# thu-nics/Rad-NeRF

Hardware: AMD Instinct MI355X
Metric: million samples/s fwd+bwd, 8192 rays, model_zoo_size=2; rgb L∞ vs ref (higher is better)
Workload: dtype f16/f32

## Files before the change

rad-nerf_amd/csrc/field.hip:

```cpp
#include "rn_field.h"
#include "rn_bin.h"
#pragma clang fp contract(off)

static int g_field_dbg = 0;
static uint64_t g_level_pairing = 0;
__device__ unsigned long long g_rn_cyc[8];

namespace {

template <int MODE, int CACHE>
__global__ void __launch_bounds__(256, FWD_MIN_WAVES)
k_field_fwd(FieldArgs a) {
    __shared__ __attribute__((aligned(16))) rn_half sW[FIELD_FWD_FRAGS * RN_FRAG_HALFS];
    __shared__ LvTab sT;
    const int k = blockIdx.y;
    rn_block_copy16(sW, a.frags + (size_t)k * FIELD_FRAGS * RN_FRAG_HALFS,
                    FIELD_FWD_FRAGS * RN_FRAG_BYTES);
    lv_stage(sT, a.gm);
    __syncthreads();
    int64_t base, n;
    sample_range(a, MODE, k, base, n);
    const int64_t n_tiles = (n + 31) / 32;
    const int waves = blockDim.x / RN_WAVE;
    const int lane = rn_lane(), h = lane >> 5;
// ... 1147 lines not shown
                              : sWm + (size_t)k * FIELD_FWD_FRAGS * RN_FRAG_HALFS;
        tile_forward_s<1, TC>(a, sT, W, s, valid, TC != CACHE_NONE ? cache_slot(a, s) : nullptr,
                              st, ux, uy, uz);
        if (valid && h == 0) {
            a.sigma[s] = expf(st.g0);
            a.rgb[3 * s + 0] = sigmoidf(st.out[0]);
            a.rgb[3 * s + 1] = sigmoidf(st.out[1]);
            a.rgb[3 * s + 2] = sigmoidf(st.out[2]);
        }
    };
    auto mlp_tiles = [&](const int32_t* ch) {
        int max_t = 0;
        for (int k = 0; k < K; ++k) max_t = max(max_t, (ch[2 + FM_KMAX + k] + 31) >> 5);
        return max_t * K;
    };

    bool prev_live = false;
    for (int it = 0;; ++it) {
        int32_t* cur = sCh[it & 1];
        const int32_t* prev = sCh[(it & 1) ^ 1];
        __syncthreads();
        if (threadIdx.x == 0) {
            const int ch = ticket;
            ticket = atomicAdd(m.queue + 2, 1);
            int4 d[CH_DESC / 4];
            if (ch < n_chunks) {
#pragma unroll
                for (int q = 0; q < CH_DESC / 4; ++q)
                    d[q] = reinterpret_cast<const int4*>(m.desc + (size_t)ch * CH_DESC)[q];
            }
            const int32_t* di = reinterpret_cast<const int32_t*>(d);
            cur[0] = ch < n_chunks ? di[0] : B;
            cur[1] = ch < n_chunks ? di[1] : B;
            for (int k = 0; k < K; ++k) {
                cur[2 + k] = di[4 + k];
                cur[2 + FM_KMAX + k] = ch < n_chunks ? di[4 + MB_KMAX + k] : 0;
            }
        }
        __syncthreads();
        const bool live = cur[0] < B;
        if (!ENC_M) {
            if (!live) break;
            const int nt = mlp_tiles(cur);
            for (int u = wid; u < nt; u += waves) mlp_tile(cur, u);
            continue;
        }
        if (!live && !prev_live) break;
        int p_base = 0, n_p = 0;
        if (live) { p_base = m.mstart[cur[0]]; n_p = m.mstart[cur[1]] - p_base; }
        const int nA = (n_p + 31) >> 5;
        const int nB = prev_live ? mlp_tiles(prev) : 0;
        for (int u = wid; u < nA + nB; u += waves) {
            if (u >= nA) { mlp_tile(prev, u - nA); continue; }
            const int q = u * 32 + c;
            const bool valid = q < n_p;
            const int64_t s = m.perm[p_base + (valid ? q : 0)];
            float x, y, z, dx, dy, dz;
            load_sample<1>(a, s, x, y, z, dx, dy, dz);
            const float ux = unit_coord(x, a.xyz_min[0], a.extent[0]);
            const float uy = unit_coord(y, a.xyz_min[1], a.extent[1]);
            const float uz = unit_coord(z, a.xyz_min[2], a.extent[2]);
            half8 e0, e1;
            encode_lane(a, sT, rn_rsrc(a.grid, a.grid_bytes), h, ux, uy, uz, valid, e0, e1);
            if (valid) { half8* fc = cache_slot(a, s); fc[0] = e0; fc[1] = e1; }
        }
        prev_live = live;
    }
}


__global__ void __launch_bounds__(256)
k_enc_prep(FieldArgs a, MergeArgs m, float4* __restrict__ prep) {
    const int P = m.mstart[m.n_rays];
    for (int p = blockIdx.x * blockDim.x + threadIdx.x; p < P; p += gridDim.x * blockDim.x) {
        const int s = m.perm[p];
        float x, y, z, dx, dy, dz;
        load_sample<1>(a, s, x, y, z, dx, dy, dz);
        prep[p] = make_float4(unit_coord(x, a.xyz_min[0], a.extent[0]),
                              unit_coord(y, a.xyz_min[1], a.extent[1]),
                              unit_coord(z, a.xyz_min[2], a.extent[2]), __int_as_float(s));
    }
}

__global__ void __launch_bounds__(256)
k_field_encode_levels(FieldArgs a, MergeArgs m, const float4* __restrict__ prep,
                      int32_t* __restrict__ xq, uint64_t pairing) {
    __shared__ LvTab sT;
    lv_stage(sT, a.gm);
    __syncthreads();
    const int g = blockIdx.x & 7;
    if (xq && threadIdx.x == 0) {
        uint32_t xcc;
        asm volatile("s_getreg_b32 %0, hwreg(HW_REG_XCC_ID, 0, 4)" : "=s"(xcc));
        atomicAdd(xq + 8 * g + (int)(xcc & 7u), 1);
        atomicMin(reinterpret_cast<unsigned long long*>(xq + 64) + g,
                  (unsigned long long)__builtin_amdgcn_s_memrealtime());
    }
    const int la = (int)((pairing >> (8 * g)) & 15u), lb = (int)((pairing >> (8 * g + 4)) & 15u);
    const int P = m.mstart[m.n_rays];
    const int nt = (P + 31) >> 5;
    const int nb = (int)(gridDim.x >> 3), j = (int)(blockIdx.x >> 3);
    const int t0 = (int)((int64_t)nt * j / nb), t1 = (int)((int64_t)nt * (j + 1) / nb);
    const int wid = __builtin_amdgcn_readfirstlane(threadIdx.x >> 6), waves = blockDim.x >> 6;
    const int lane = rn_lane(), c = lane & 31, h = lane >> 5;
    const __amdgpu_buffer_rsrc_t rs = rn_rsrc(a.grid, a.grid_bytes);
    const LvConst LA = lv_const_uniform(sT, a.gm, la), LB = lv_const_uniform(sT, a.gm, lb);
#pragma unroll 1
    for (int ph = 0; ph < 2; ++ph) {
        const LvConst& LC = ph ? LB : LA;
        uint32_t* const out = const_cast<uint32_t*>(a.planes) + (size_t)(ph ? lb : la) * a.plane_stride;
        for (int t = t0 + 2 * wid; t < t1; t += 2 * waves) {
            const bool v0 = t * 32 + c < P;
            const bool v1 = t + 1 < t1 && (t + 1) * 32 + c < P;
            const bool valid = h ? v1 : v0;
            const int p = (t + h) * 32 + c;
            const float4 q = prep[valid ? p : 0];
            const uint32_t v = encode_tiles(a, rs, h, LC, q.x, q.y, q.z, v0, v1);
            if (valid) __builtin_nontemporal_store(v, out + __float_as_int(q.w));
        }
    }
    if (xq) {
        __syncthreads();
        if (threadIdx.x == 0)
            atomicMax(reinterpret_cast<unsigned long long*>(xq + 80) + g,
                      (unsigned long long)__builtin_amdgcn_s_memrealtime());
    }
}

__global__ void __launch_bounds__(1024)
k_field_mlp_planes(FieldArgs a, int K) {
    extern __shared__ __attribute__((aligned(16))) rn_half sWm[];
    __shared__ LvTab sT;
    __shared__ int32_t sSeg[2][FM_KMAX];
    lv_stage(sT, a.gm);
    if (threadIdx.x < K) {
        sSeg[0][threadIdx.x] = a.seg_base[threadIdx.x];
        sSeg[1][threadIdx.x] = a.seg_count[threadIdx.x];
    }
    int first[FM_KMAX + 1];
    first[0] = 0;
    for (int k = 0; k < K; ++k)
        first[k + 1] = first[k] + ((__builtin_amdgcn_readfirstlane(a.seg_count[k]) + 31) >> 5);
    const int T = first[K];
    const int u0 = (int)((int64_t)T * blockIdx.x / gridDim.x);
    const int u1 = (int)((int64_t)T * (blockIdx.x + 1) / gridDim.x);
    if (u0 >= u1) return;
    int k_lo = 0, k_hi = 0;
    for (int k = 0; k < K; ++k) {
        if (first[k + 1] <= u0) k_lo = k + 1;
        if (first[k] < u1) k_hi = k;
    }
    const int wid = __builtin_amdgcn_readfirstlane(threadIdx.x >> 6), waves = blockDim.x >> 6;
    const int lane = rn_lane(), c = lane & 31, h = lane >> 5;
    for (int kb = k_lo; kb <= k_hi; kb += FM_LDS_K) {
        const int ke = min(k_hi, kb + FM_LDS_K - 1);
        __syncthreads();
        for (int k = kb; k <= ke; ++k)
            rn_block_copy16(sWm + (size_t)(k - kb) * FIELD_FWD_FRAGS * RN_FRAG_HALFS,
                            a.frags + (size_t)k * FIELD_FRAGS * RN_FRAG_HALFS,
                            FIELD_FWD_FRAGS * RN_FRAG_BYTES);
        __syncthreads();
        const int ua = max(u0, first[kb]), ub = min(u1, first[ke + 1]);
        for (int u = ua + wid; u < ub; u += waves) {
            int k = kb;
            while (k < ke && u >= first[k + 1]) ++k;
            const int t = u - first[k];
            const int n_k = sSeg[1][k];
            const int i = t * 32 + c;
            const bool valid = i < n_k;
            const int64_t s = sSeg[0][k] + (valid ? i : 0);
            FwdState st;
            float ux, uy, uz;
            rn_lds_order();
            tile_forward_s<1, CACHE_PLANES>(a, sT, sWm + (size_t)(k - kb) * FIELD_FWD_FRAGS * RN_FRAG_HALFS,
                                            s, valid, a.feat ? cache_slot(a, s) : nullptr, st,
                                            ux, uy, uz);
            if (valid && h == 0) {
                a.sigma[s] = expf(st.g0);
                a.rgb[3 * s + 0] = sigmoidf(st.out[0]);
                a.rgb[3 * s + 1] = sigmoidf(st.out[1]);
                a.rgb[3 * s + 2] = sigmoidf(st.out[2]);
            }
        }
    }
}


__global__ void __launch_bounds__(256)
k_seed_max(const int32_t* __restrict__ seg_base, const int32_t* __restrict__ seg_count,
           const float* __restrict__ sigma, const float* __restrict__ dsigma,
           const float* __restrict__ drgb, uint32_t* __restrict__ mbits) {
    const int k = blockIdx.y;
    const int64_t base = seg_base[k], n = seg_count[k];
    float mx = 0.f;
    for (int64_t i = (int64_t)blockIdx.x * blockDim.x + threadIdx.x; i < n;
         i += (int64_t)gridDim.x * blockDim.x) {
        const int64_t s = base + i;
        mx = fmaxf(mx, fabsf(dsigma[s] * sigma[s]));
        mx = fmaxf(mx, fmaxf(fabsf(drgb[3 * s]), fmaxf(fabsf(drgb[3 * s + 1]), fabsf(drgb[3 * s + 2]))));
    }
    mx = rn_wave_max(mx);
    if (rn_lane() == 0 && mx > 0.f && isfinite(mx)) atomicMax(mbits, __float_as_uint(mx));
// ... 793 lines not shown
        }
    }
    if (fx_mode == 5) {
        k_field_bwd_merged<CACHE_READ, false, 5><<<blocks, blk, 0, st>>>(a, m, G, F);
    } else if (fx_mode == 4) {
        k_field_bwd_merged<CACHE_READ, false, 4><<<blocks, blk, 0, st>>>(a, m, G, F);
    } else if (fx_mode == 2) {
        k_field_bwd_merged<CACHE_READ, false, 2><<<blocks, blk, 0, st>>>(a, m, G, F);
    } else if (fx_mode == 3) {
        k_field_bwd_merged<CACHE_READ, false, 3><<<blocks, blk, 0, st>>>(a, m, G, F);
    } else if (igrad_lo) {
        if (feat_cache) k_field_bwd_merged<CACHE_READ, false, 1><<<blocks, blk, 0, st>>>(a, m, G, F);
        else k_field_bwd_merged<CACHE_NONE, false, 1><<<blocks, blk, 0, st>>>(a, m, G, F);
    } else {
        if (feat_cache) k_field_bwd_merged<CACHE_READ, false, 0><<<blocks, blk, 0, st>>>(a, m, G, F);
        else k_field_bwd_merged<CACHE_NONE, false, 0><<<blocks, blk, 0, st>>>(a, m, G, F);
    }
    RN_CHECK_LAUNCH();
    return 0;
}

int rn_field_fwd_merged(const float* ts, const int32_t* ray_of, const float* rays_o,
                        const float* rays_d, const int32_t* seg_base, const int32_t* seg_count,
                        const int32_t* chunk_desc, int32_t* queue,
                        int64_t n_rays, int32_t n_models, const void* grid_f16,
                        const uint32_t* level_offset, const uint32_t* level_hsize,
                        const uint32_t* level_res, const float* level_scale,
                        const float* xyz_min, const float* extent, const void* frags,
                        float* sigma, float* rgb, void* feat_cache, const int32_t* mstart,
                        const int32_t* perm, int32_t blocks, int32_t threads, void* stream) {
    RN_CHECK_ARG(n_rays >= 1 && n_models >= 1 && n_models <= FM_KMAX && blocks >= 1,
                 "bad sizes (n_models <= 8)");
    RN_CHECK_ARG(threads >= 64 && threads <= 1024 && threads % 64 == 0, "threads: 64..1024, waves");
    RN_CHECK_ARG(ts && ray_of && rays_o && rays_d && seg_base && seg_count &&
                 chunk_desc && queue && grid_f16 && level_offset && level_hsize && level_res &&
                 level_scale && xyz_min && extent && frags && sigma && rgb, "null pointer");
    RN_CHECK_ARG(!(mstart || perm) || (mstart && perm && feat_cache),
                 "merged-order encoding needs mstart, perm and the encoding cache");
    FieldArgs a{};
    fill_args(a, xyz_min, extent, level_offset, level_hsize, level_res, level_scale);
    a.dbg = rn_dbg(g_field_dbg);
    a.grid = (const rn_half*)grid_f16; a.frags = (const rn_half*)frags;
    a.sigma = sigma; a.rgb = rgb; a.feat = (rn_half*)feat_cache;
    a.ts = ts; a.ray_of = ray_of; a.rays_o = rays_o; a.rays_d = rays_d;
    a.seg_base = seg_base; a.seg_count = seg_count;
    MergeArgs m{};
    m.desc = chunk_desc; m.queue = queue;
    m.mstart = mstart; m.perm = perm;
    m.n_rays = (int)n_rays; m.n_models = n_models;
    const bool gw = n_models > FM_LDS_K;
    const size_t lds = gw ? 0 : (size_t)n_models * FIELD_FWD_FRAGS * RN_FRAG_BYTES;
    hipStream_t st = (hipStream_t)stream;
    if (hipMemsetAsync(queue + 2, 0, sizeof(int32_t), st) != hipSuccess) {
        rn_set_error("%s: ticket reset failed", __func__);
        return 2;
    }
#define RN_FM_LAUNCH(C, E)                                                                     \
    do {                                                                                       \
        if (gw) k_field_fwd_merged<C, E, true><<<blocks, threads, 0, st>>>(a, m);              \
        else k_field_fwd_merged<C, E, false><<<blocks, threads, lds, st>>>(a, m);              \
    } while (0)
    if (mstart) RN_FM_LAUNCH(CACHE_WRITE, true);
    else if (feat_cache) RN_FM_LAUNCH(CACHE_WRITE, false);
    else RN_FM_LAUNCH(CACHE_NONE, false);
#undef RN_FM_LAUNCH
    RN_CHECK_LAUNCH();
    return 0;
}

int rn_field_fwd_levels(const float* ts, const int32_t* ray_of, const float* rays_o,
                        const float* rays_d, const int32_t* seg_base, const int32_t* seg_count,
                        int64_t n_rays, int32_t n_models, const void* grid_f16,
                        const uint32_t* level_offset, const uint32_t* level_hsize,
                        const uint32_t* level_res, const float* level_scale,
                        const float* xyz_min, const float* extent, const void* frags,
                        float* sigma, float* rgb, void* feat_cache, const int32_t* mstart,
                        const int32_t* perm, uint32_t* planes, int64_t plane_stride, void* prep,
                        int32_t prep_ready, int32_t enc_blocks, int32_t mlp_blocks, int32_t* xq,
                        void* stream) {
    RN_CHECK_ARG(n_rays >= 1 && n_models >= 1 && n_models <= FM_KMAX && plane_stride >= 1,
                 "bad sizes (n_models <= 8)");
    RN_CHECK_ARG(enc_blocks >= 8 && enc_blocks % 8 == 0 && mlp_blocks >= 1,
                 "bad launch (enc_blocks: a multiple of 8)");
    RN_CHECK_ARG(ts && ray_of && rays_o && rays_d && seg_base && seg_count && grid_f16 &&
                 level_offset && level_hsize && level_res && level_scale && xyz_min && extent &&
                 frags && sigma && rgb && mstart && perm && planes && prep, "null pointer");
    FieldArgs a{};
    fill_args(a, xyz_min, extent, level_offset, level_hsize, level_res, level_scale);
    a.dbg = rn_dbg(g_field_dbg);
    a.grid = (const rn_half*)grid_f16; a.frags = (const rn_half*)frags;
    a.sigma = sigma; a.rgb = rgb; a.feat = (rn_half*)feat_cache;
    a.planes = planes; a.plane_stride = plane_stride;
    a.ts = ts; a.ray_of = ray_of; a.rays_o = rays_o; a.rays_d = rays_d;
    a.seg_base = seg_base; a.seg_count = seg_count;
    MergeArgs m{};
    m.mstart = mstart; m.perm = perm; m.n_rays = (int)n_rays; m.n_models = n_models;
    hipStream_t st = (hipStream_t)stream;
    if (xq && (hipMemsetAsync(xq, 0, 64 * sizeof(int32_t), st) != hipSuccess ||
               hipMemsetAsync(xq + 64, 0xff, 16 * sizeof(int32_t), st) != hipSuccess ||
               hipMemsetAsync(xq + 80, 0, 16 * sizeof(int32_t), st) != hipSuccess)) {
        rn_set_error("%s: probe reset failed", __func__);
        return 2;
    }
    if (!prep_ready) k_enc_prep<<<1024, 256, 0, st>>>(a, m, (float4*)prep);
    uint64_t pairing = g_level_pairing;
    if (pairing == 0)
        for (int g = 0; g < 8; ++g) pairing |= (uint64_t)(g | ((RN_L - 1 - g) << 4)) << (8 * g);
    k_field_encode_levels<<<enc_blocks, 256, 0, st>>>(a, m, (const float4*)prep, xq, pairing);
    k_field_mlp_planes<<<mlp_blocks, 1024,
                         (size_t)min(n_models, FM_LDS_K) * FIELD_FWD_FRAGS * RN_FRAG_BYTES, st>>>(
        a, n_models);
    RN_CHECK_LAUNCH();
    return 0;
}

int rn_seed_scale(const int32_t* seg_base, const int32_t* seg_count, int32_t n_models,
                  const float* sigma, const float* dL_dsigma, const float* dL_drgb,
                  uint32_t* work, float* scale, void* stream) {
    RN_CHECK_ARG(n_models >= 1, "bad sizes");
    RN_CHECK_ARG(seg_base && seg_count && sigma && dL_dsigma && dL_drgb && work && scale,
                 "null pointer");
    hipStream_t st = (hipStream_t)stream;
    if (hipMemsetAsync(work, 0, sizeof(uint32_t), st) != hipSuccess) {
        rn_set_error("%s: memset failed", __func__);
        return 2;
    }
    k_seed_max<<<dim3(256, n_models), 256, 0, st>>>(seg_base, seg_count, sigma, dL_dsigma,
                                                     dL_drgb, work);
    RN_CHECK_LAUNCH();
    k_seed_scale<<<1, 1, 0, st>>>(work, scale);
    RN_CHECK_LAUNCH();
    return 0;
}

int rn_grid_fx_fold(const uint32_t* level_offset, const uint32_t* level_hsize,
                    const uint32_t* level_res, int32_t* fx_acc, const float* fx_scale_cur,
                    float* fx_scale_next, uint32_t* fx_vmax, int32_t* fx_redo, float* grid_grad,
                    void* stream) {
    RN_CHECK_ARG(level_offset && level_hsize && level_res && fx_acc && fx_scale_cur &&
                 fx_scale_next && fx_vmax && fx_redo && grid_grad, "null pointer");
    RN_CHECK_ARG(fx_scale_cur != fx_scale_next, "scale_cur and scale_next must differ");
    GridMeta gm{};
    uint32_t hashed = 0;
    for (int l = 0; l < RN_L; ++l) {
        gm.offset[l] = level_offset[l]; gm.hsize[l] = level_hsize[l]; gm.res[l] = level_res[l];
        const uint64_t r = level_res[l];
        if (r * r * r > (uint64_t)level_hsize[l]) hashed |= 1u << l;
        RN_CHECK_ARG(level_offset[l] % 8 == 0, "level offsets must be multiples of 8 entries");
    }
    hipStream_t st = (hipStream_t)stream;
    FxStats* stats = reinterpret_cast<FxStats*>(fx_vmax);
    k_fx_esum<<<dim3(128, RN_L), 256, 0, st>>>(gm, fx_scale_cur, fx_acc, grid_grad, stats);
    k_fx_check<<<1, 64, 0, st>>>(hashed, fx_scale_cur, fx_scale_next, stats, fx_redo, nullptr, 0u);
    RN_CHECK_LAUNCH();
    {
        const int64_t e0 = 2 * (int64_t)level_offset[0];
        const int64_t e1 = 2 * ((int64_t)level_offset[RN_L - 1] + level_hsize[RN_L - 1]);
        RN_CHECK_ARG(e1 % 4 == 0, "table size must be a multiple of 2 entries");
        const int64_t n4 = (e1 - e0) / 4;
        const int nb = (int)std::min<int64_t>(2048, (n4 + 255) / 256);
        k_fx_fold<<<nb > 0 ? nb : 1, 256, 0, st>>>(e0, e1, gm, fx_scale_cur, fx_acc, grid_grad,
                                                    fx_redo);
        RN_CHECK_LAUNCH();
    }
    return 0;
}
// ... 27 lines not shown
```

rad-nerf_amd/csrc/rn_field.h:

```cpp
#pragma once
#include "rn_mlp.h"
#pragma clang fp contract(off)

#define RN_L 16
#define FIELD_FWD_FRAGS 24
#define FIELD_FRAGS 46
#define FIELD_PARAMS 9472
#define FIELD_DW_TILES 12
#ifndef FWD_MIN_WAVES
#define FWD_MIN_WAVES 2
#endif

struct GridMeta {
    uint32_t offset[RN_L];
    uint32_t hsize[RN_L];
    uint32_t res[RN_L];
    float scale[RN_L];
    uint32_t dense_mask;
    uint32_t pow2_mask;
};

struct FieldArgs {
    const float* xyzs; const float* dirs;
    const float* ts; const int32_t* ray_of; const float* rays_o; const float* rays_d;
// ... 135 lines not shown
                for (int r = 0; r < 4; ++r)
                    rw[r] = b + ((r & 1) ? lm.res : 0u) + ((r >> 1) ? lm.res2 : 0u);
            } else {
                const uint32_t y0 = p.gy * 2654435761u, z0 = p.gz * 805459861u;
                const uint32_t y1 = y0 + 2654435761u, z1 = z0 + 805459861u;
#pragma unroll
                for (int r = 0; r < 4; ++r) rw[r] = ((r & 1) ? y1 : y0) ^ ((r >> 1) ? z1 : z0);
            }
            auto xch = [&](uint32_t v, uint32_t& lo, uint32_t& hi) {
                const auto r2 = __builtin_amdgcn_permlane32_swap(v, v, false, false);
                lo = r2[0]; hi = r2[1];
            };
            uint32_t t0, t1;
            xch(p.gx, GX[up], GX[up + 1]);
            xch(__float_as_uint(p.fx), t0, t1); FX[up] = __uint_as_float(t0); FX[up + 1] = __uint_as_float(t1);
            xch(__float_as_uint(p.fy), t0, t1); FY[up] = __uint_as_float(t0); FY[up + 1] = __uint_as_float(t1);
            xch(__float_as_uint(p.fz), t0, t1); FZ[up] = __uint_as_float(t0); FZ[up + 1] = __uint_as_float(t1);
#pragma unroll
            for (int r = 0; r < 4; ++r) xch(rw[r], ROW[up][r], ROW[up + 1][r]);
        }
        uint32_t off[16];
#pragma unroll
        for (int u = 0; u < 4; ++u) {
            const LvConst lc = lv_const(T, a.gm, lb + u);
            const uint32_t x = GX[u] + (uint32_t)h;
            uint32_t idx[4];
            if (lc.dense) {
#pragma unroll
                for (int r = 0; r < 4; ++r) {
                    const uint32_t d = x + ROW[u][r];
                    idx[r] = min(d, d - lc.hs);
                }
            } else {
#pragma unroll
                for (int r = 0; r < 4; ++r) idx[r] = (x ^ ROW[u][r]) & (lc.hs - 1u);
            }
            const uint32_t ob = load ? lc.off : (RN_OOB >> 2);
#pragma unroll
            for (int r = 0; r < 4; ++r) off[4 * u + r] = (ob + idx[r]) << 2;
        }
        uint32_t raw[16];
#pragma unroll
        for (int i = 0; i < 16; ++i) raw[i] = __builtin_amdgcn_raw_buffer_load_b32(rs, off[i], 0, 0);
#pragma unroll
        for (int u = 0; u < 4; ++u) {
            float a0 = 0.f, a1 = 0.f;
            const float wx = h ? FX[u] : 1.0f - FX[u];
            const float wy0 = 1.0f - FY[u], wz0 = 1.0f - FZ[u];
            const float wxy0 = wx * wy0, wxy1 = wx * FY[u];
#pragma unroll
            for (int r = 0; r < 4; ++r) {
                const float w = ((r & 1) ? wxy1 : wxy0) * ((r >> 1) ? FZ[u] : wz0);
                const uint32_t v = raw[4 * u + r];
                a0 = fmaf(w, (float)__builtin_bit_cast(rn_half, (uint16_t)(v & 0xffffu)), a0);
                a1 = fmaf(w, (float)__builtin_bit_cast(rn_half, (uint16_t)(v >> 16)), a1);
            }
            const auto s0 = __builtin_amdgcn_permlane32_swap(__float_as_uint(a0), __float_as_uint(a0), false, false);
            const auto s1 = __builtin_amdgcn_permlane32_swap(__float_as_uint(a1), __float_as_uint(a1), false, false);
            const float v0 = __uint_as_float(s0[0]) + __uint_as_float(s0[1]);
            const float v1 = __uint_as_float(s1[0]) + __uint_as_float(s1[1]);
            const int L = lb + u, q = (L & 1) + 2 * (L >> 2);
            if (((L >> 1) & 1) == h) { f[2 * q] = v0; f[2 * q + 1] = v1; }
        }
#ifndef FWD_NO_SCHED_BARRIER
        __builtin_amdgcn_sched_barrier(0);
#endif
    }
#pragma unroll
    for (int j = 0; j < 8; ++j) { e0[j] = (rn_half)f[j]; e1[j] = (rn_half)f[8 + j]; }
}

__device__ __forceinline__ LvConst lv_const_uniform(const LvTab& T, const GridMeta& gm, int l) {
    const LvConst c = lv_const(T, gm, l);
    LvConst u;
    u.off = (uint32_t)__builtin_amdgcn_readfirstlane((int)c.off);
    u.hs = (uint32_t)__builtin_amdgcn_readfirstlane((int)c.hs);
    u.res = (uint32_t)__builtin_amdgcn_readfirstlane((int)c.res);
    u.res2 = (uint32_t)__builtin_amdgcn_readfirstlane((int)c.res2);
    u.sc = __int_as_float(__builtin_amdgcn_readfirstlane(__float_as_int(c.sc)));
    u.dense = c.dense;
    return u;
}

__device__ __forceinline__ uint32_t encode_tiles(const FieldArgs& a, __amdgpu_buffer_rsrc_t rs,
                                                 int h, const LvConst& L, float ux, float uy,
                                                 float uz, bool valid0, bool valid1) {
    uint32_t GX[2], ROW[2][4];
    float FX[2], FY[2], FZ[2];
    const int dn = __builtin_amdgcn_readfirstlane((int)L.dense);
    {
        const LevelPos p = level_pos(L.sc, ux, uy, uz);
        uint32_t rw[4];
        if (dn) {
            const uint32_t b = __umul24(p.gy, L.res) + __umul24(p.gz, L.res2);
#pragma unroll
            for (int r = 0; r < 4; ++r) rw[r] = b + ((r & 1) ? L.res : 0u) + ((r >> 1) ? L.res2 : 0u);
        } else {
            const uint32_t y0 = p.gy * 2654435761u, z0 = p.gz * 805459861u;
            const uint32_t y1 = y0 + 2654435761u, z1 = z0 + 805459861u;
#pragma unroll
            for (int r = 0; r < 4; ++r) rw[r] = ((r & 1) ? y1 : y0) ^ ((r >> 1) ? z1 : z0);
        }
        auto xch = [&](uint32_t v, uint32_t& lo, uint32_t& hi) {
            const auto r2 = __builtin_amdgcn_permlane32_swap(v, v, false, false);
            lo = r2[0]; hi = r2[1];
        };
        uint32_t t0, t1;
        xch(p.gx, GX[0], GX[1]);
        xch(__float_as_uint(p.fx), t0, t1); FX[0] = __uint_as_float(t0); FX[1] = __uint_as_float(t1);
        xch(__float_as_uint(p.fy), t0, t1); FY[0] = __uint_as_float(t0); FY[1] = __uint_as_float(t1);
        xch(__float_as_uint(p.fz), t0, t1); FZ[0] = __uint_as_float(t0); FZ[1] = __uint_as_float(t1);
#pragma unroll
        for (int r = 0; r < 4; ++r) xch(rw[r], ROW[0][r], ROW[1][r]);
    }
    const bool noload = rn_dbg(a.dbg) & 128;
    uint32_t off[8];
#pragma unroll
    for (int u = 0; u < 2; ++u) {
        const uint32_t x = GX[u] + (uint32_t)h;
        const uint32_t ob = ((u ? valid1 : valid0) && !noload) ? L.off : (RN_OOB >> 2);
        if (dn) {
#pragma unroll
            for (int r = 0; r < 4; ++r) {
                const uint32_t d = x + ROW[u][r];
                off[4 * u + r] = (ob + min(d, d - L.hs)) << 2;
            }
        } else {
#pragma unroll
            for (int r = 0; r < 4; ++r) off[4 * u + r] = (ob + ((x ^ ROW[u][r]) & (L.hs - 1u))) << 2;
        }
    }
    uint32_t raw[8];
#pragma unroll
    for (int i = 0; i < 8; ++i) raw[i] = __builtin_amdgcn_raw_buffer_load_b32(rs, off[i], 0, 0);
    uint32_t res = 0u;
#pragma unroll
    for (int u = 0; u < 2; ++u) {
        float a0 = 0.f, a1 = 0.f;
        const float wx = h ? FX[u] : 1.0f - FX[u];
        const float wy0 = 1.0f - FY[u], wz0 = 1.0f - FZ[u];
        const float wxy0 = wx * wy0, wxy1 = wx * FY[u];
#pragma unroll
        for (int r = 0; r < 4; ++r) {
            const float w = ((r & 1) ? wxy1 : wxy0) * ((r >> 1) ? FZ[u] : wz0);
            const uint32_t v = raw[4 * u + r];
            a0 = fmaf(w, (float)__builtin_bit_cast(rn_half, (uint16_t)(v & 0xffffu)), a0);
            a1 = fmaf(w, (float)__builtin_bit_cast(rn_half, (uint16_t)(v >> 16)), a1);
        }
        const auto s0 = __builtin_amdgcn_permlane32_swap(__float_as_uint(a0), __float_as_uint(a0), false, false);
        const auto s1 = __builtin_amdgcn_permlane32_swap(__float_as_uint(a1), __float_as_uint(a1), false, false);
        const float v0 = __uint_as_float(s0[0]) + __uint_as_float(s0[1]);
        const float v1 = __uint_as_float(s1[0]) + __uint_as_float(s1[1]);
        const uint32_t pk = (uint32_t)__builtin_bit_cast(uint16_t, (rn_half)v0) |
                            ((uint32_t)__builtin_bit_cast(uint16_t, (rn_half)v1) << 16);
        if (u == h) res = pk;
    }
    return res;
}

__device__ __forceinline__ half8 sh_lane(float dx, float dy, float dz, int h) {
    const float n = sqrtf(dx * dx + dy * dy + dz * dz);
    const float x = fmaf((dx / n + 1.0f) / 2.0f, 2.0f, -1.0f);
    const float y = fmaf((dy / n + 1.0f) / 2.0f, 2.0f, -1.0f);
    const float z = fmaf((dz / n + 1.0f) / 2.0f, 2.0f, -1.0f);
    const float xy = x * y, xz = x * z, yz = y * z, x2 = x * x, y2 = y * y, z2 = z * z;
    float o[16];
    o[0] = 0.28209479177387814f;
    o[1] = -0.48860251190291987f * y;
    o[2] = 0.48860251190291987f * z;
    o[3] = -0.48860251190291987f * x;
    o[4] = 1.0925484305920792f * xy;
    o[5] = -1.0925484305920792f * yz;
    o[6] = 0.94617469575755997f * z2 - 0.31539156525251999f;
    o[7] = -1.0925484305920792f * xz;
    o[8] = 0.54627421529603959f * x2 - 0.54627421529603959f * y2;
    o[9] = 0.59004358992664352f * y * (-3.0f * x2 + y2);
    o[10] = 2.8906114426405538f * xy * z;
    o[11] = 0.45704579946446572f * y * (1.0f - 5.0f * z2);
    o[12] = 0.3731763325901154f * z * (5.0f * z2 - 3.0f);
    o[13] = 0.45704579946446572f * x * (1.0f - 5.0f * z2);
    o[14] = 1.4453057213202769f * z * (x2 - y2);
    o[15] = 0.59004358992664352f * x * (-x2 + 3.0f * y2);
    half8 r;
#pragma unroll
    for (int j = 0; j < 8; ++j) {
        const int c0 = 8 * (j >> 2) + (j & 3);
        r[j] = (rn_half)(h ? o[c0 + 4] : o[c0]);
    }
    return r;
}

struct FwdState {
    half8 e0, e1;
    half8 h1[4];
    half8 gin;
    half8 sh;
    half8 r1[4], r2[4];
    float g0;
    f32x16 out;
};

__device__ __forceinline__ void mlp_forward(const rn_half* W, FwdState& st) {
    f32x16 a0 = rn_zero16(), a1 = rn_zero16();
    a0 = rn_mfma(rn_frag(W, 0), st.e0, a0); a0 = rn_mfma(rn_frag(W, 1), st.e1, a0);
    a1 = rn_mfma(rn_frag(W, 2), st.e0, a1); a1 = rn_mfma(rn_frag(W, 3), st.e1, a1);
    rn_acc_to_frags<true>(a0, st.h1[0], st.h1[1]);
    rn_acc_to_frags<true>(a1, st.h1[2], st.h1[3]);
    f32x16 g = rn_zero16();
#pragma unroll
    for (int q = 0; q < 4; ++q) g = rn_mfma(rn_frag(W, 4 + q), st.h1[q], g);
    half8 gk1;
    rn_acc_to_frags<false>(g, st.gin, gk1);
    st.g0 = g[8];
    a0 = rn_zero16(); a1 = rn_zero16();
    a0 = rn_mfma(rn_frag(W, 8), st.sh, a0); a0 = rn_mfma(rn_frag(W, 9), st.gin, a0);
    a1 = rn_mfma(rn_frag(W, 10), st.sh, a1); a1 = rn_mfma(rn_frag(W, 11), st.gin, a1);
    rn_acc_to_frags<true>(a0, st.r1[0], st.r1[1]);
    rn_acc_to_frags<true>(a1, st.r1[2], st.r1[3]);
    a0 = rn_zero16(); a1 = rn_zero16();
#pragma unroll
    for (int q = 0; q < 4; ++q) {
        a0 = rn_mfma(rn_frag(W, 12 + q), st.r1[q], a0);
        a1 = rn_mfma(rn_frag(W, 16 + q), st.r1[q], a1);
    }
    rn_acc_to_frags<true>(a0, st.r2[0], st.r2[1]);
    rn_acc_to_frags<true>(a1, st.r2[2], st.r2[3]);
    st.out = rn_zero16();
#pragma unroll
    for (int q = 0; q < 4; ++q) st.out = rn_mfma(rn_frag(W, 20 + q), st.r2[q], st.out);
}

__device__ __forceinline__ float sigmoidf(float x) { return 1.0f / (1.0f + expf(-x)); }

enum { CACHE_NONE = 0, CACHE_WRITE = 1, CACHE_READ = 2,
       CACHE_READ_NT = 3,
       CACHE_PLANES = 4 };

template <int CACHE>
__device__ __forceinline__ void tile_forward_pos(const FieldArgs& a, const LvTab& T, const rn_half* W,
                                                 float x, float y, float z, float dx, float dy,
                                                 float dz, bool valid, half8* fc, FwdState& st,
                                                 float& ux, float& uy, float& uz);

template <int MODE, int CACHE>
__device__ __forceinline__ void tile_forward_s(const FieldArgs& a, const LvTab& T, const rn_half* W,
                                               int64_t s, bool valid, half8* fc, FwdState& st,
                                               float& ux, float& uy, float& uz) {
    float x = 0.f, y = 0.f, z = 0.f, dx = 1.f, dy = 0.f, dz = 0.f;
    if (CACHE == CACHE_PLANES) {
        const int h = rn_lane() >> 5;
        typedef uint32_t u4v __attribute__((ext_vector_type(4)));
        u4v w0 = {0u, 0u, 0u, 0u}, w1 = {0u, 0u, 0u, 0u};
        if (valid) {
            const uint32_t* pl = a.planes + s;
#pragma unroll
            for (int q = 0; q < 4; ++q) {
                w0[q] = pl[(size_t)lane_level(q, h) * a.plane_stride];
                w1[q] = pl[(size_t)lane_level(q + 4, h) * a.plane_stride];
            }
        }
        st.e0 = __builtin_bit_cast(half8, w0); st.e1 = __builtin_bit_cast(half8, w1);
    }
    if (valid) load_sample<MODE>(a, s, x, y, z, dx, dy, dz);
    tile_forward_pos<CACHE>(a, T, W, x, y, z, dx, dy, dz, valid, fc, st, ux, uy, uz);
}

template <int CACHE>
__device__ __forceinline__ void tile_forward_rays(const FieldArgs& a, const LvTab& T,
                                                  const rn_half* W, int64_t s, bool valid,
                                                  half8* fc, const float* sRays, int r0, int nr,
                                                  FwdState& st, float& ux, float& uy, float& uz) {
    float x = 0.f, y = 0.f, z = 0.f, dx = 1.f, dy = 0.f, dz = 0.f;
    if (valid) {
        const int r = a.ray_of[s];
        const float t = a.ts[s];
        const uint32_t q = (uint32_t)(r - r0);
        float ox, oy, oz;
        if (q < (uint32_t)nr) {
            typedef __attribute__((address_space(3))) const float lds_f;
            lds_f* p = (lds_f*)sRays + 6 * q;
            ox = p[0]; oy = p[1]; oz = p[2]; dx = p[3]; dy = p[4]; dz = p[5];
        } else {
            ox = a.rays_o[3 * r]; oy = a.rays_o[3 * r + 1]; oz = a.rays_o[3 * r + 2];
            dx = a.rays_d[3 * r]; dy = a.rays_d[3 * r + 1]; dz = a.rays_d[3 * r + 2];
        }
        x = fmaf(t, dx, ox);
        y = fmaf(t, dy, oy);
        z = fmaf(t, dz, oz);
    }
    tile_forward_pos<CACHE>(a, T, W, x, y, z, dx, dy, dz, valid, fc, st, ux, uy, uz);
}

template <int CACHE>
__device__ __forceinline__ void tile_forward_pos(const FieldArgs& a, const LvTab& T, const rn_half* W,
                                                 float x, float y, float z, float dx, float dy,
                                                 float dz, bool valid, half8* fc, FwdState& st,
                                                 float& ux, float& uy, float& uz) {
    const int h = rn_lane() >> 5;
    ux = unit_coord(x, a.xyz_min[0], a.extent[0]);
    uy = unit_coord(y, a.xyz_min[1], a.extent[1]);
    uz = unit_coord(z, a.xyz_min[2], a.extent[2]);
    if (CACHE == CACHE_PLANES) {
        if (valid && fc) { fc[0] = st.e0; fc[1] = st.e1; }
    } else if (CACHE == CACHE_READ || CACHE == CACHE_READ_NT) {
        st.e0 = rn_zero8(); st.e1 = rn_zero8();
        if (valid && CACHE == CACHE_READ) { st.e0 = fc[0]; st.e1 = fc[1]; }
        if (valid && CACHE == CACHE_READ_NT) {
            st.e0 = __builtin_nontemporal_load(fc);
            st.e1 = __builtin_nontemporal_load(fc + 1);
        }
    } else {
        if (rn_dbg(a.dbg) & 256) { st.e0 = rn_zero8(); st.e1 = rn_zero8(); asm volatile("" :: "v"(ux), "v"(uy), "v"(uz)); }
        else encode_lane(a, T, rn_rsrc(a.grid, a.grid_bytes), h, ux, uy, uz, valid, st.e0, st.e1);
        if (CACHE == CACHE_WRITE && valid) { fc[0] = st.e0; fc[1] = st.e1; }
    }
    st.sh = sh_lane(dx, dy, dz, h);
    if (rn_dbg(a.dbg) & 4096) {
        st.out = rn_zero16(); st.g0 = 0.f;
        asm volatile("" :: "v"(st.e0), "v"(st.e1), "v"(st.sh));
    } else {
        mlp_forward(W, st);
    }
}

__device__ __forceinline__ half8* cache_slot(const FieldArgs& a, int64_t s) {
    return reinterpret_cast<half8*>(a.feat) + ((s >> 5) * 64 + (s & 31) + 32 * (rn_lane() >> 5)) * 2;
}

template <int MODE, int CACHE>
__device__ __forceinline__ void tile_forward(const FieldArgs& a, const LvTab& T, const rn_half* W,
                                             int64_t base, int64_t n, int64_t tile, FwdState& st,
                                             bool& valid, int64_t& s, float& ux, float& uy,
                                             float& uz) {
    const int lane = rn_lane(), c = lane & 31;
    const int64_t i = tile * 32 + c;
    valid = i < n;
// ... 24 lines not shown
```

Before: 1194.

## Specialize level encoder on dense/full tiles and use byte-offset buffer loads

Templates the hash-grid encode on dense versus hashed levels and on full tiles, precomputes byte-scaled strides so the per-corner offset math drops the final shift and the valid selects, and rebases the buffer resource per level so bounds checks cover only that level. The bilinear weights are computed in packed two-wide vectors, and the final cross-half reduction is merged into fewer permlane swaps with a packed f16 convert. The plane gather in the MLP path now uses buffer loads with scalar level offsets. These changes target VALU and SGPR overhead in the encode and gather kernels, at the cost of extra code paths and a new 32-bit limit on plane offsets.

```diff
diff --git a/rad-nerf_amd/csrc/field.hip b/rad-nerf_amd/csrc/field.hip
--- a/rad-nerf_amd/csrc/field.hip
+++ b/rad-nerf_amd/csrc/field.hip
@@ -1253,6 +1253,35 @@
     }
 }
 
+template <bool DENSE>
+__device__ __forceinline__ void encode_level_pass(__amdgpu_buffer_rsrc_t rs, const LvBytes& L,
+                                                  const float4* __restrict__ prep,
+                                                  uint32_t* __restrict__ out, int t0, int t1,
+                                                  int P, int wid, int waves, int c, int h) {
+    const uint32_t lo = (uint32_t)(h * 32 + c) * 16u;
+    auto row = [&](int t, uint32_t o) {
+        return *reinterpret_cast<const float4*>(reinterpret_cast<const char*>(prep + (size_t)t * 32) + o);
+    };
+    auto put = [&](uint32_t v, float sw) {
+        const uint32_t so = (uint32_t)__float_as_int(sw) << 2;
+        __builtin_nontemporal_store(v, reinterpret_cast<uint32_t*>(reinterpret_cast<char*>(out) + so));
+    };
+    int t = t0 + 2 * wid;
+    auto full = [&](int u) { return u + 1 < t1 && (u + 2) * 32 <= P; };
+    for (; full(t); t += 2 * waves) {
+        const float4 q = row(t, lo);
+        put(encode_tiles<DENSE, true>(rs, h, L, q.x, q.y, q.z, true, true), q.w);
+    }
+    for (; t < t1; t += 2 * waves) {
+        const bool v0 = t * 32 + c < P;
+        const bool v1 = t + 1 < t1 && (t + 1) * 32 + c < P;
+        const bool valid = h ? v1 : v0;
+        const float4 q = row(t, valid ? lo : 0u);
+        const uint32_t v = encode_tiles<DENSE, false>(rs, h, L, q.x, q.y, q.z, v0, v1);
+        if (valid) put(v, q.w);
+    }
+}
+
 __global__ void __launch_bounds__(256)
 k_field_encode_levels(FieldArgs a, MergeArgs m, const float4* __restrict__ prep,
                       int32_t* __restrict__ xq, uint64_t pairing) {
@@ -1268,27 +1297,26 @@
                   (unsigned long long)__builtin_amdgcn_s_memrealtime());
     }
     const int la = (int)((pairing >> (8 * g)) & 15u), lb = (int)((pairing >> (8 * g + 4)) & 15u);
-    const int P = m.mstart[m.n_rays];
+    const int P = __builtin_amdgcn_readfirstlane(m.mstart[m.n_rays]);
     const int nt = (P + 31) >> 5;
     const int nb = (int)(gridDim.x >> 3), j = (int)(blockIdx.x >> 3);
     const int t0 = (int)((int64_t)nt * j / nb), t1 = (int)((int64_t)nt * (j + 1) / nb);
     const int wid = __builtin_amdgcn_readfirstlane(threadIdx.x >> 6), waves = blockDim.x >> 6;
     const int lane = rn_lane(), c = lane & 31, h = lane >> 5;
-    const __amdgpu_buffer_rsrc_t rs = rn_rsrc(a.grid, a.grid_bytes);
-    const LvConst LA = lv_const_uniform(sT, a.gm, la), LB = lv_const_uniform(sT, a.gm, lb);
 #pragma unroll 1
     for (int ph = 0; ph < 2; ++ph) {
-        const LvConst& LC = ph ? LB : LA;
-        uint32_t* const out = const_cast<uint32_t*>(a.planes) + (size_t)(ph ? lb : la) * a.plane_stride;
-        for (int t = t0 + 2 * wid; t < t1; t += 2 * waves) {
-            const bool v0 = t * 32 + c < P;
-            const bool v1 = t + 1 < t1 && (t + 1) * 32 + c < P;
-            const bool valid = h ? v1 : v0;
-            const int p = (t + h) * 32 + c;
-            const float4 q = prep[valid ? p : 0];
-            const uint32_t v = encode_tiles(a, rs, h, LC, q.x, q.y, q.z, v0, v1);
-            if (valid) __builtin_nontemporal_store(v, out + __float_as_int(q.w));
-        }
+        const int lv = __builtin_amdgcn_readfirstlane(ph ? lb : la);
+        const LvConst LC = lv_const_uniform(sT, a.gm, lv);
+        uint32_t* const out = const_cast<uint32_t*>(a.planes) + (size_t)lv * a.plane_stride;
+        const uint32_t lv0 = 4u * LC.off;
+        const uint32_t room = a.grid_bytes > lv0 ? a.grid_bytes - lv0 : 0u;
+        const uint32_t lvb = (uint32_t)__builtin_amdgcn_readfirstlane(
+            (int)(4u * LC.hs < room ? 4u * LC.hs : room));
+        const __amdgpu_buffer_rsrc_t rs = rn_rsrc(reinterpret_cast<const char*>(a.grid) + lv0,
+                                                  (rn_dbg(a.dbg) & 128) ? 0u : lvb);
+        const LvBytes L = lv_bytes(LC);
+        if (LC.dense) encode_level_pass<true>(rs, L, prep, out, t0, t1, P, wid, waves, c, h);
+        else encode_level_pass<false>(rs, L, prep, out, t0, t1, P, wid, waves, c, h);
     }
     if (xq) {
         __syncthreads();
@@ -2248,6 +2276,7 @@
                  "bad sizes (n_models <= 8)");
     RN_CHECK_ARG(enc_blocks >= 8 && enc_blocks % 8 == 0 && mlp_blocks >= 1,
                  "bad launch (enc_blocks: a multiple of 8)");
+    RN_CHECK_ARG(plane_stride <= ((int64_t)1 << 30), "plane_stride above 2^30 (32-bit plane offsets)");
     RN_CHECK_ARG(ts && ray_of && rays_o && rays_d && seg_base && seg_count && grid_f16 &&
                  level_offset && level_hsize && level_res && level_scale && xyz_min && extent &&
                  frags && sigma && rgb && mstart && perm && planes && prep, "null pointer");
diff --git a/rad-nerf_amd/csrc/rn_field.h b/rad-nerf_amd/csrc/rn_field.h
--- a/rad-nerf_amd/csrc/rn_field.h
+++ b/rad-nerf_amd/csrc/rn_field.h
@@ -241,22 +241,39 @@
     return u;
 }
 
-__device__ __forceinline__ uint32_t encode_tiles(const FieldArgs& a, __amdgpu_buffer_rsrc_t rs,
-                                                 int h, const LvConst& L, float ux, float uy,
-                                                 float uz, bool valid0, bool valid1) {
+struct LvBytes {
+    uint32_t res4, res24;
+    uint32_t hs4;
+    uint32_t mask4;
+    float sc;
+};
+
+__device__ __forceinline__ LvBytes lv_bytes(const LvConst& u) {
+    LvBytes b;
+    b.res4 = u.res << 2; b.res24 = u.res2 << 2; b.hs4 = u.hs << 2; b.mask4 = (u.hs - 1u) << 2;
+    b.sc = u.sc;
+    return b;
+}
+
+template <bool DENSE, bool FULL>
+__device__ __forceinline__ uint32_t encode_tiles(__amdgpu_buffer_rsrc_t rs, int h, const LvBytes& L,
+                                                 float ux, float uy, float uz, bool valid0,
+                                                 bool valid1) {
+    typedef float vf2 __attribute__((ext_vector_type(2)));
+    typedef _Float16 vh2 __attribute__((ext_vector_type(2)));
     uint32_t GX[2], ROW[2][4];
-    float FX[2], FY[2], FZ[2];
-    const int dn = __builtin_amdgcn_readfirstlane((int)L.dense);
+    vf2 FX, FY, FZ;
     {
         const LevelPos p = level_pos(L.sc, ux, uy, uz);
         uint32_t rw[4];
-        if (dn) {
-            const uint32_t b = __umul24(p.gy, L.res) + __umul24(p.gz, L.res2);
-#pragma unroll
-            for (int r = 0; r < 4; ++r) rw[r] = b + ((r & 1) ? L.res : 0u) + ((r >> 1) ? L.res2 : 0u);
+        if (DENSE) {
+            const uint32_t b = __umul24(p.gy, L.res4) + __umul24(p.gz, L.res24);
+#pragma unroll
+            for (int r = 0; r < 4; ++r) rw[r] = b + ((r & 1) ? L.res4 : 0u) + ((r >> 1) ? L.res24 : 0u);
         } else {
-            const uint32_t y0 = p.gy * 2654435761u, z0 = p.gz * 805459861u;
-            const uint32_t y1 = y0 + 2654435761u, z1 = z0 + 805459861u;
+            constexpr uint32_t P1 = 2654435761u * 4u, P2 = 805459861u * 4u;
+            const uint32_t y0 = p.gy * P1, z0 = p.gz * P2;
+            const uint32_t y1 = y0 + P1, z1 = z0 + P2;
 #pragma unroll
             for (int r = 0; r < 4; ++r) rw[r] = ((r & 1) ? y1 : y0) ^ ((r >> 1) ? z1 : z0);
         }
@@ -264,57 +281,58 @@
             const auto r2 = __builtin_amdgcn_permlane32_swap(v, v, false, false);
             lo = r2[0]; hi = r2[1];
         };
-        uint32_t t0, t1;
+        auto xchf = [&](float v, vf2& o) {
+            uint32_t t0, t1;
+            xch(__float_as_uint(v), t0, t1);
+            o[0] = __uint_as_float(t0); o[1] = __uint_as_float(t1);
+        };
         xch(p.gx, GX[0], GX[1]);
-        xch(__float_as_uint(p.fx), t0, t1); FX[0] = __uint_as_float(t0); FX[1] = __uint_as_float(t1);
-        xch(__float_as_uint(p.fy), t0, t1); FY[0] = __uint_as_float(t0); FY[1] = __uint_as_float(t1);
-        xch(__float_as_uint(p.fz), t0, t1); FZ[0] = __uint_as_float(t0); FZ[1] = __uint_as_float(t1);
+        xchf(p.fx, FX); xchf(p.fy, FY); xchf(p.fz, FZ);
 #pragma unroll
         for (int r = 0; r < 4; ++r) xch(rw[r], ROW[0][r], ROW[1][r]);
     }
-    const bool noload = rn_dbg(a.dbg) & 128;
     uint32_t off[8];
 #pragma unroll
     for (int u = 0; u < 2; ++u) {
-        const uint32_t x = GX[u] + (uint32_t)h;
-        const uint32_t ob = ((u ? valid1 : valid0) && !noload) ? L.off : (RN_OOB >> 2);
-        if (dn) {
-#pragma unroll
-            for (int r = 0; r < 4; ++r) {
-                const uint32_t d = x + ROW[u][r];
-                off[4 * u + r] = (ob + min(d, d - L.hs)) << 2;
+        const uint32_t x4 = (GX[u] + (uint32_t)h) << 2;
+#pragma unroll
+        for (int r = 0; r < 4; ++r) {
+            uint32_t o;
+            if (DENSE) {
+                const uint32_t d4 = x4 + ROW[u][r];
+                o = min(d4, d4 - L.hs4);
+            } else {
+                o = (x4 ^ ROW[u][r]) & L.mask4;
             }
-        } else {
-#pragma unroll
-            for (int r = 0; r < 4; ++r) off[4 * u + r] = (ob + ((x ^ ROW[u][r]) & (L.hs - 1u))) << 2;
+            if (!FULL) o = (u ? valid1 : valid0) ? o : RN_OOB;
+            off[4 * u + r] = o;
         }
     }
     uint32_t raw[8];
 #pragma unroll
     for (int i = 0; i < 8; ++i) raw[i] = __builtin_amdgcn_raw_buffer_load_b32(rs, off[i], 0, 0);
-    uint32_t res = 0u;
+    const float sg = h ? 1.0f : -1.0f, bs = h ? 0.0f : 1.0f;
+    const vf2 one = {1.0f, 1.0f};
+    const vf2 wx = {fmaf(FX[0], sg, bs), fmaf(FX[1], sg, bs)};
+    const vf2 wy0 = one - FY, wz0 = one - FZ;
+    const vf2 wxy0 = wx * wy0, wxy1 = wx * FY;
+    const vf2 w[4] = {wxy0 * wz0, wxy1 * wz0, wxy0 * FZ, wxy1 * FZ};
+    uint32_t S[2];
 #pragma unroll
     for (int u = 0; u < 2; ++u) {
         float a0 = 0.f, a1 = 0.f;
-        const float wx = h ? FX[u] : 1.0f - FX[u];
-        const float wy0 = 1.0f - FY[u], wz0 = 1.0f - FZ[u];
-        const float wxy0 = wx * wy0, wxy1 = wx * FY[u];
 #pragma unroll
         for (int r = 0; r < 4; ++r) {
-            const float w = ((r & 1) ? wxy1 : wxy0) * ((r >> 1) ? FZ[u] : wz0);
             const uint32_t v = raw[4 * u + r];
-            a0 = fmaf(w, (float)__builtin_bit_cast(rn_half, (uint16_t)(v & 0xffffu)), a0);
-            a1 = fmaf(w, (float)__builtin_bit_cast(rn_half, (uint16_t)(v >> 16)), a1);
-        }
-        const auto s0 = __builtin_amdgcn_permlane32_swap(__float_as_uint(a0), __float_as_uint(a0), false, false);
-        const auto s1 = __builtin_amdgcn_permlane32_swap(__float_as_uint(a1), __float_as_uint(a1), false, false);
-        const float v0 = __uint_as_float(s0[0]) + __uint_as_float(s0[1]);
-        const float v1 = __uint_as_float(s1[0]) + __uint_as_float(s1[1]);
-        const uint32_t pk = (uint32_t)__builtin_bit_cast(uint16_t, (rn_half)v0) |
-                            ((uint32_t)__builtin_bit_cast(uint16_t, (rn_half)v1) << 16);
-        if (u == h) res = pk;
-    }
-    return res;
+            a0 = fmaf(w[r][u], (float)__builtin_bit_cast(rn_half, (uint16_t)(v & 0xffffu)), a0);
+            a1 = fmaf(w[r][u], (float)__builtin_bit_cast(rn_half, (uint16_t)(v >> 16)), a1);
+        }
+        const auto s = __builtin_amdgcn_permlane32_swap(__float_as_uint(a0), __float_as_uint(a1), false, false);
+        S[u] = __float_as_uint(__uint_as_float(s[0]) + __uint_as_float(s[1]));
+    }
+    const auto f = __builtin_amdgcn_permlane32_swap(S[0], S[1], false, false);
+    const vf2 fv = {__uint_as_float(f[0]), __uint_as_float(f[1])};
+    return __builtin_bit_cast(uint32_t, __builtin_convertvector(fv, vh2));
 }
 
 __device__ __forceinline__ half8 sh_lane(float dx, float dy, float dz, int h) {
@@ -410,7 +428,16 @@
         const int h = rn_lane() >> 5;
         typedef uint32_t u4v __attribute__((ext_vector_type(4)));
         u4v w0 = {0u, 0u, 0u, 0u}, w1 = {0u, 0u, 0u, 0u};
-        if (valid) {
+        if (valid && a.plane_stride < ((int64_t)1 << 26)) {
+            const uint32_t st4 = (uint32_t)a.plane_stride << 2;
+            const __amdgpu_buffer_rsrc_t pr = rn_rsrc(a.planes, 16u * st4);
+            const uint32_t vo = ((uint32_t)s << 2) + (uint32_t)(2 * h) * st4;
+#pragma unroll
+            for (int q = 0; q < 4; ++q) {
+                w0[q] = __builtin_amdgcn_raw_buffer_load_b32(pr, vo, (uint32_t)lane_level(q, 0) * st4, 0);
+                w1[q] = __builtin_amdgcn_raw_buffer_load_b32(pr, vo, (uint32_t)lane_level(q + 4, 0) * st4, 0);
+            }
+        } else if (valid) {
             const uint32_t* pl = a.planes + s;
 #pragma unroll
             for (int q = 0; q < 4; ++q) {
```

Result: no change. 1197, median of 3 (+0.3%).
